# wfus/Fully-Homomorphic-Image-Processing

Measured on AMD Instinct MI355X. Metric: encrypted 8x8 blocks/sec (homomorphic DCT+quant), higher is better.
Workload: dtype f64

## Files before the change

fully-homomorphic-image-processing_amd/csrc/dct_fused.hip:

```cpp
#include "internal.h"

#include <cstdlib>

#include "fp64_core.h"

#pragma clang fp contract(off)

namespace {
using namespace fp64;

template <int L, int LE> struct Shape {
    static constexpr int N = 1 << L, E = 1 << LE, TP = N >> LE, NP = (L + LE - 1) / LE, LDS_WORDS = N + (N >> LE);
};
__host__ __device__ constexpr int g_lo(int L, int LE, int p) { return (L - LE * p - LE) < 0 ? 0 : (L - LE * p - LE); }
__host__ __device__ constexpr int g_stages(int L, int LE, int p) { return (L - LE * p) > LE ? LE : (L - LE * p); }
template <int LO, int LE> __device__ __forceinline__ int g_index(int tid, int r) {
    return ((tid >> LO) << (LO + LE)) | (r << LO) | (tid & ((1 << LO) - 1));
}
template <int LO, int LE> __device__ __forceinline__ int g_pad(int j) { return j + ((j >> (LO + LE)) << LO); }

template <int L, int LE, int P> struct PassTw {
    static constexpr int LO = g_lo(L, LE, P), S = g_stages(L, LE, P), NTW = (1 << LE) - 1;
    static constexpr int rb(int u) { return (L - 1 - (LE * P + u)) - LO; }
    static constexpr int count(int u) { return 1 << (LE - 1 - rb(u)); }
    static constexpr int offset(int u) { int o = 0; for (int v = 0; v < u; v++) o += count(v); return o; }
};
template <int L, int LE, int P>
__device__ __forceinline__ void load_tw(double (&w)[(1 << LE) - 1], const double *__restrict__ tw, int tid) {
    using T = PassTw<L, LE, P>;
    const int th = (P == 0) ? 0 : (tid >> T::LO);
#pragma unroll
    for (int u = 0; u < T::S; u++) {
#pragma unroll
        for (int i = 0; i < T::count(u); i++) w[T::offset(u) + i] = tw[(1 << (LE * P + u)) + ((th << (LE - 1 - T::rb(u))) | i)];
    }
}

template <int L, int LE, int P, int M>
__device__ __forceinline__ void fwd_pass(double (&x)[M][1 << LE], const double (&w)[(1 << LE) - 1], double p, double pinv) {
    using T = PassTw<L, LE, P>;
    constexpr int E = 1 << LE, KB = (LE == 3) ? 2 : 1;
#pragma unroll
    for (int u = 0; u < T::S; u++) {
        const int rb = T::rb(u);
#pragma unroll
        for (int b0 = 0; b0 < E / 2; b0 += KB) {
            double t[KB * M], wm[KB * M];
#pragma unroll
            for (int kb = 0; kb < KB; kb++) {
                const int b = b0 + kb, r0 = ((b >> rb) << (rb + 1)) | (b & ((1 << rb) - 1)), r1 = r0 | (1 << rb);
                const double wv = w[T::offset(u) + (r0 >> (rb + 1))];
#pragma unroll
                for (int m = 0; m < M; m++) { t[kb * M + m] = x[m][r1]; wm[kb * M + m] = wv; }
            }
            mmv<KB * M>(t, wm, p, pinv);
#pragma unroll
            for (int kb = 0; kb < KB; kb++) {
                const int b = b0 + kb, r0 = ((b >> rb) << (rb + 1)) | (b & ((1 << rb) - 1)), r1 = r0 | (1 << rb);
#pragma unroll
                for (int m = 0; m < M; m++) {
                    const double X = x[m][r0];
                    x[m][r0] = X + t[kb * M + m];
                    x[m][r1] = X - t[kb * M + m];
                }
            }
        }
    }
}

template <int L, int LE, int P, int M>
__device__ __forceinline__ void inv_pass(double (&x)[M][1 << LE], const double (&w)[(1 << LE) - 1], double ninv, double p, double pinv) {
    using T = PassTw<L, LE, P>;
    constexpr int E = 1 << LE, KB = (LE == 3) ? 2 : 1;
#pragma unroll
    for (int u = T::S - 1; u >= 0; u--) {
        const int sigma = LE * P + u, rb = T::rb(u);
        if (sigma == 0) {
#pragma unroll
            for (int b = 0; b < E / 2; b++) {
                const int r0 = ((b >> rb) << (rb + 1)) | (b & ((1 << rb) - 1)), r1 = r0 | (1 << rb);
                const double wv = w[T::offset(u) + (r0 >> (rb + 1))];
                double t[2 * M], wm[2 * M];
#pragma unroll
                for (int m = 0; m < M; m++) {
                    const double X = x[m][r0], Y = x[m][r1];
                    t[m] = X + Y; wm[m] = ninv;
                    t[M + m] = X - Y; wm[M + m] = wv;
                }
                mmv<2 * M>(t, wm, p, pinv);
#pragma unroll
                for (int m = 0; m < M; m++) { x[m][r0] = t[m]; x[m][r1] = t[M + m]; }
            }
        } else {
#pragma unroll
            for (int b0 = 0; b0 < E / 2; b0 += KB) {
                double t[KB * M], wm[KB * M];
#pragma unroll
                for (int kb = 0; kb < KB; kb++) {
                    const int b = b0 + kb, r0 = ((b >> rb) << (rb + 1)) | (b & ((1 << rb) - 1)), r1 = r0 | (1 << rb);
                    const double wv = w[T::offset(u) + (r0 >> (rb + 1))];
#pragma unroll
                    for (int m = 0; m < M; m++) {
                        const double X = x[m][r0], Y = x[m][r1];
                        x[m][r0] = X + Y;
                        t[kb * M + m] = X - Y; wm[kb * M + m] = wv;
                    }
                }
                mmv<KB * M>(t, wm, p, pinv);
#pragma unroll
                for (int kb = 0; kb < KB; kb++) {
                    const int b = b0 + kb, r0 = ((b >> rb) << (rb + 1)) | (b & ((1 << rb) - 1)), r1 = r0 | (1 << rb);
#pragma unroll
                    for (int m = 0; m < M; m++) x[m][r1] = t[kb * M + m];
                }
            }
        }
    }
}

template <int L, int LE, int LO_FROM, int LO_TO, int M>
__device__ __forceinline__ void transpose(double (&x)[M][1 << LE], double *lds, int tid, int &phase) {
    constexpr int PL = imin(LO_FROM, LO_TO), E = 1 << LE;
    constexpr bool WAVE_LOCAL = (Shape<L, LE>::TP <= 64) || (LO_FROM <= 6 && LO_TO <= 6);
#pragma unroll
    for (int m = 0; m < M; m++) {
        double *buf = lds + (phase & 1) * Shape<L, LE>::LDS_WORDS;
        phase++;
#pragma unroll
        for (int r = 0; r < E; r++) buf[g_pad<PL, LE>(g_index<LO_FROM, LE>(tid, r))] = x[m][r];
        if constexpr (WAVE_LOCAL) {
            __builtin_amdgcn_fence(__ATOMIC_RELEASE, "wavefront");
            __builtin_amdgcn_wave_barrier();
            __builtin_amdgcn_fence(__ATOMIC_ACQUIRE, "wavefront");
        } else {
            __syncthreads();
        }
#pragma unroll
        for (int r = 0; r < E; r++) x[m][r] = buf[g_pad<PL, LE>(g_index<LO_TO, LE>(tid, r))];
    }
}

template <int L, int LE, int M, typename PRE, int P = 0>
__device__ __forceinline__ void ntt_fwd(double (&x)[M][1 << LE], double (&w)[(1 << LE) - 1], const double *__restrict__ tw, double p, double pinv,
                                        double *lds, int tid, int &phase, PRE pre) {
    if constexpr (P + 1 < Shape<L, LE>::NP) {
        double wn[(1 << LE) - 1];
        if (LE >= 4) load_tw<L, LE, P + 1>(wn, tw, tid);
        fwd_pass<L, LE, P, M>(x, w, p, pinv);
        if (LE < 4) load_tw<L, LE, P + 1>(wn, tw, tid);
        if constexpr (P + 2 == Shape<L, LE>::NP) pre();
        transpose<L, LE, g_lo(L, LE, P), g_lo(L, LE, P + 1), M>(x, lds, tid, phase);
        ntt_fwd<L, LE, M, PRE, P + 1>(x, wn, tw, p, pinv, lds, tid, phase, pre);
    } else {
        fwd_pass<L, LE, P, M>(x, w, p, pinv);
    }
}
template <int L, int LE, int M, bool BIG, int P = Shape<L, LE>::NP - 1>
__device__ __forceinline__ void ntt_inv(double (&x)[M][1 << LE], double (&w)[(1 << LE) - 1], const double *__restrict__ itw, double p, double pinv,
                                        double *lds, int tid, int &phase) {
    if constexpr (P > 0) {
        double wn[(1 << LE) - 1];
        if (LE >= 4) load_tw<L, LE, P - 1>(wn, itw, tid);
        inv_pass<L, LE, P, M>(x, w, 0.0, p, pinv);
        if (LE < 4) load_tw<L, LE, P - 1>(wn, itw, tid);
        if constexpr (BIG) {
#pragma unroll
            for (int m = 0; m < M; m++)
#pragma unroll
                for (int r = 0; r < (1 << LE); r++) x[m][r] = red(x[m][r], p, pinv);
        }
        transpose<L, LE, g_lo(L, LE, P), g_lo(L, LE, P - 1), M>(x, lds, tid, phase);
        ntt_inv<L, LE, M, BIG, P - 1>(x, wn, itw, p, pinv, lds, tid, phase);
    } else {
        inv_pass<L, LE, P, M>(x, w, itw[0], p, pinv);
    }
}

constexpr double PACK_BIAS = 6755399441055744.0;
template <int E, int TP>
__device__ __forceinline__ void store_packed(u64 *__restrict__ o, const double (&x)[E]) {
    static_assert(E == 8, "packed layout is defined for 8 values per thread");
    u32 lo[8], hi[8];
#pragma unroll
    for (int r = 0; r < 8; r++) {
        const double t = x[r] + PACK_BIAS;
        lo[r] = (u32)__double2loint(t);
        hi[r] = (u32)__double2hiint(t);
    }
#pragma unroll
    for (int q = 0; q < 4; q++) o[q * TP] = (u64)lo[2 * q] | ((u64)lo[2 * q + 1] << 32);
    u32 h[2];
#pragma unroll
    for (int g = 0; g < 2; g++) {
        const u32 p01 = __builtin_amdgcn_perm(hi[4 * g + 1], hi[4 * g + 0], 0x0c0c0400u);
        const u32 p23 = __builtin_amdgcn_perm(hi[4 * g + 3], hi[4 * g + 2], 0x0c0c0400u);
        h[g] = __builtin_amdgcn_perm(p23, p01, 0x05040100u);
    }
    o[4 * TP] = (u64)h[0] | ((u64)h[1] << 32);
}
typedef __attribute__((address_space(1))) const void lc_gptr;
typedef __attribute__((address_space(3))) void lc_lptr;
template <int NT>
__device__ __forceinline__ void stage_consts(const char *ubase, u32 voff, size_t cstride_bytes, double *stg, int lane) {
#pragma unroll
    for (int i0 = 0; i0 < NT; i0 += 2) {
        const int i = (i0 + 1 < NT) ? i0 : NT - 2;
        const char *b = ubase + (size_t)i * cstride_bytes;
        __builtin_amdgcn_global_load_lds((lc_gptr *)(b + voff), (lc_lptr *)(stg + i * 64), 16, 0, 0);
    }
}

template <int L, int LE, bool BIG, int HALF, bool PACK, bool LDSC>
__device__ __forceinline__ void rows_body(const u64 *__restrict__ in, double *__restrict__ mid, const double *__restrict__ consts,
                                          const double *__restrict__ tw, const Work &wk, double p, double pinv, u32 k, double *lds) {
    using SH = Shape<L, LE>;
    constexpr int N = SH::N, TP = SH::TP, E = SH::E, NC = HalfC<HALF>::NC, FIRST = HalfC<HALF>::FIRST;
    const int tid = threadIdx.x;
    const size_t poly_words = (size_t)k * N, ct_words = 2 * poly_words;
    const size_t base = ((size_t)wk.blk * 64 + 8 * wk.line) * ct_words + (size_t)wk.poly * poly_words + (size_t)wk.prime * N;
    double w0[E - 1];
    load_tw<L, LE, 0>(w0, tw, tid);
    double x[4][E];
    constexpr u64 OFF = 1ULL << 48;
    u64 ra[2][E], rb[2][E];
    auto issue = [&](int m) {
        const u64 *a = in + base + (size_t)m * ct_words + tid, *b = in + base + (size_t)(7 - m) * ct_words + tid;
#pragma unroll
        for (int r = 0; r < E; r++) {
            ra[m & 1][r] = a[r * TP];
            rb[m & 1][r] = b[r * TP];
        }
    };
    auto combine = [&](int m) {
#pragma unroll
        for (int r = 0; r < E; r++) {
            const u64 A = ra[m & 1][r], B = rb[m & 1][r];
            x[m][r] = HALF ? u52_to_f64(A + OFF - B) - (double)OFF : u52_to_f64(A + B);
        }
    };
    if constexpr (LE >= 4) {
        issue(0);
        issue(1);
        asm volatile("" ::: "memory");
        combine(0);
        issue(2);
        asm volatile("" ::: "memory");
        combine(1);
        issue(3);
        asm volatile("" ::: "memory");
        combine(2);
        combine(3);
    } else {
#pragma unroll
        for (int m = 0; m < 4; m++) {
            issue(m);
            combine(m);
            asm volatile("" ::: "memory");
        }
    }
    const double *cp = consts + (size_t)FIRST * k * N + (size_t)wk.prime * N + tid;
    const size_t cstride = (size_t)k * N;
    double cn[9];
    auto fetch = [&](int r) {
#pragma unroll
        for (int i = 0; i < NC; i++) cn[i] = cp[(size_t)i * cstride + r * TP];
    };
    int phase = 0;
    ntt_fwd<L, LE, 4>(x, w0, tw, p, pinv, lds, tid, phase, [&] { if (LE >= 4) fetch(0); });
    const int lane = tid & 63;
    double *stg = lds + (tid >> 6) * (2 * NC * 64);
    const char *sbase = (const char *)(consts + (size_t)FIRST * cstride + (size_t)wk.prime * N);
    const u32 svoff = (u32)(((size_t)(lane >> 5) * cstride + (tid & ~63) + 2 * (lane & 31)) * sizeof(double));
    constexpr int NDMA = (NC + 1) / 2;
    if constexpr (LDSC) {
        __syncthreads();
        stage_consts<NC>(sbase, svoff, cstride * sizeof(double), stg, lane);
    }
#pragma unroll
    for (int r = 0; r < E; r++) {
        double c[9];
        if constexpr (LDSC) {
            if (r + 1 < E) stage_consts<NC>(sbase + (size_t)(r + 1) * TP * sizeof(double), svoff, cstride * sizeof(double), stg + ((r + 1) & 1) * NC * 64, lane);
            if (r + 1 < E) asm volatile("s_waitcnt vmcnt(%0)" ::"n"(NDMA) : "memory");
            else asm volatile("s_waitcnt vmcnt(0)" ::: "memory");
            const double *sr = stg + (r & 1) * NC * 64 + lane;
#pragma unroll
            for (int i = 0; i < NC; i++) c[i] = sr[i * 64];
        } else {
        if (LE < 4) fetch(r);
#pragma unroll
        for (int i = 0; i < NC; i++) c[i] = cn[i];
        if (LE >= 4 && r + 1 < E) fetch(r + 1);
        }
        line_half<HALF>(x[0][r], x[1][r], x[2][r], x[3][r], c, p, pinv);
        if (BIG) {
#pragma unroll
            for (int m = 0; m < 4; m++) x[m][r] = red(x[m][r], p, pinv);
        } else if (PACK && HALF == 0) {
            x[0][r] = red(x[0][r], p, pinv);
            x[2][r] = red(x[2][r], p, pinv);
        }
        if constexpr (LDSC) asm volatile("" ::"v"(x[0][r]), "v"(x[1][r]), "v"(x[2][r]), "v"(x[3][r]) : "memory");
    }
#pragma unroll
    for (int m = 0; m < 4; m++) {
        double *o = mid + base + (size_t)(2 * m + HALF) * ct_words + tid;
        if constexpr (PACK) {
            store_packed<E, TP>((u64 *)o, x[m]);
        } else {
#pragma unroll
            for (int r = 0; r < E; r++) o[r * TP] = x[m][r];
        }
    }
}

__host__ __device__ constexpr int occ_waves(int tp, int lds_words) {
    return ((2 * lds_words * 16 <= 160 * 1024) ? 2 : 1) * tp / 256 < 1 ? 1 : ((2 * lds_words * 16 <= 160 * 1024) ? 2 : 1) * tp / 256;
}
template <int L, int LE> struct Occ { static constexpr int W = occ_waves(Shape<L, LE>::TP, Shape<L, LE>::LDS_WORDS); };

template <int L, int LE, bool BIG, bool PACK, bool LDSC>
__global__ __launch_bounds__((Shape<L, LE>::TP), (Occ<L, LE>::W)) void k_dct_rows(const u64 *__restrict__ in, double *__restrict__ mid,
                                                                  const double *__restrict__ consts, const double *__restrict__ tw_all,
                                                                  const Modulus *__restrict__ mods, u32 k) {
    __shared__ double lds[2 * Shape<L, LE>::LDS_WORDS];
    const Work wk = decode(blockIdx.x, k);
    const double p = (double)mods[wk.prime].q, pinv = 1.0 / p;
    const double *tw = tw_all + (size_t)wk.prime * Shape<L, LE>::N;
    if (wk.half) rows_body<L, LE, BIG, 1, PACK, LDSC>(in, mid, consts, tw, wk, p, pinv, k, lds);
    else rows_body<L, LE, BIG, 0, PACK, LDSC>(in, mid, consts, tw, wk, p, pinv, k, lds);
}

template <int L, int LE, bool BIG, int HALF, bool PACK>
__device__ __forceinline__ void cols_body(const double *__restrict__ mid, u64 *__restrict__ out, const double *__restrict__ consts,
                                          const double *__restrict__ itw, const Work &wk, double p, double pinv, u32 k, double *lds) {
    using SH = Shape<L, LE>;
    constexpr int N = SH::N, TP = SH::TP, E = SH::E, NC = HalfC<HALF>::NC, FIRST = HalfC<HALF>::FIRST;
    constexpr int LASTP = SH::NP - 1;
    const int tid = threadIdx.x;
    const size_t poly_words = (size_t)k * N, ct_words = 2 * poly_words;
    const size_t base = ((size_t)wk.blk * 64 + wk.line) * ct_words + (size_t)wk.poly * poly_words + (size_t)wk.prime * N;
    const size_t row_stride = 8 * ct_words;
    const size_t cstride = (size_t)k * N;
    const double *cp = consts + (size_t)FIRST * cstride + (size_t)wk.prime * N + tid;
    const double *sp = consts + (size_t)(12 + 8 * HALF + wk.line) * cstride + (size_t)wk.prime * N + tid;
    double cn[9], sn[4];
    auto fetch = [&](int r) {
#pragma unroll
        for (int i = 0; i < NC; i++) cn[i] = cp[(size_t)i * cstride + r * TP];
#pragma unroll
        for (int m = 0; m < 4; m++) sn[m] = sp[(size_t)(16 * m) * cstride + r * TP];
    };
    double wl[E - 1];
    if constexpr (!PACK) {
        fetch(0);
        load_tw<L, LE, LASTP>(wl, itw, tid);
    }
    double x[4][E];
    if constexpr (PACK) {
        u64 wa[4][5], wb[4][5];
#pragma unroll
        for (int m = 0; m < 4; m++) {
            const u64 *a = (const u64 *)(mid + base + (size_t)m * row_stride) + tid, *b = (const u64 *)(mid + base + (size_t)(7 - m) * row_stride) + tid;
#pragma unroll
            for (int q = 0; q < 5; q++) { wa[m][q] = a[q * TP]; wb[m][q] = b[q * TP]; }
        }
#pragma unroll
        for (int m = 0; m < 4; m++) {
#pragma unroll
            for (int r = 0; r < E; r++) {
                const u32 la = (r & 1) ? (u32)(wa[m][r >> 1] >> 32) : (u32)wa[m][r >> 1];
                const u32 lb = (r & 1) ? (u32)(wb[m][r >> 1] >> 32) : (u32)wb[m][r >> 1];
                const u32 hwa = (r & 4) ? (u32)(wa[m][4] >> 32) : (u32)wa[m][4], hwb = (r & 4) ? (u32)(wb[m][4] >> 32) : (u32)wb[m][4];
                const double ta = __hiloint2double((int)(0x43380000u + (u32)(int)(signed char)(hwa >> (8 * (r & 3)))), (int)la);
                const double tb = __hiloint2double((int)(0x43380000u + (u32)(int)(signed char)(hwb >> (8 * (r & 3)))), (int)lb);
                x[m][r] = HALF ? ta - tb : ta + (tb - 2.0 * PACK_BIAS);
            }
        }
    } else {
#pragma unroll
        for (int m = 0; m < 4; m++) {
            const double *a = mid + base + (size_t)m * row_stride + tid, *b = mid + base + (size_t)(7 - m) * row_stride + tid;
#pragma unroll
            for (int r = 0; r < E; r++) {
                const double A = a[r * TP], B = b[r * TP];
                x[m][r] = HALF ? A - B : A + B;
            }
        }
    }
    if constexpr (PACK) load_tw<L, LE, LASTP>(wl, itw, tid);
#pragma unroll
    for (int r = 0; r < E; r++) {
        double c[9], sc[4];
        if (PACK) fetch(r);
#pragma unroll
        for (int i = 0; i < NC; i++) c[i] = cn[i];
#pragma unroll
        for (int m = 0; m < 4; m++) sc[m] = sn[m];
        if (!PACK && r + 1 < E) fetch(r + 1);
        line_half<HALF>(x[0][r], x[1][r], x[2][r], x[3][r], c, p, pinv);
        double y[4] = {x[0][r], x[1][r], x[2][r], x[3][r]};
        mmv<4>(y, sc, p, pinv);
#pragma unroll
        for (int m = 0; m < 4; m++) x[m][r] = y[m];
    }
    int phase = 0;
    ntt_inv<L, LE, 4, BIG>(x, wl, itw, p, pinv, lds, tid, phase);
#pragma unroll
    for (int m = 0; m < 4; m++) {
        u64 *o = out + base + (size_t)(2 * m + HALF) * row_stride + tid;
#pragma unroll
        for (int r = 0; r < E; r++) {
            double v = x[m][r];
            v = v < 0.0 ? v + p : v;
            o[r * TP] = f64_to_u52(v);
        }
    }
}

template <int L, int LE, bool BIG, bool PACK>
__global__ __launch_bounds__((Shape<L, LE>::TP), (Occ<L, LE>::W)) void k_dct_cols(const double *__restrict__ mid, u64 *__restrict__ out,
                                                                  const double *__restrict__ consts, const double *__restrict__ itw_all,
                                                                  const Modulus *__restrict__ mods, u32 k) {
    __shared__ double lds[2 * Shape<L, LE>::LDS_WORDS];
    const Work wk = decode(blockIdx.x, k);
    const double p = (double)mods[wk.prime].q, pinv = 1.0 / p;
    const double *itw = itw_all + (size_t)wk.prime * Shape<L, LE>::N;
    if (wk.half) cols_body<L, LE, BIG, 1, PACK>(mid, out, consts, itw, wk, p, pinv, k, lds);
    else cols_body<L, LE, BIG, 0, PACK>(mid, out, consts, itw, wk, p, pinv, k, lds);
}

template <int L, int LE>
__global__ __launch_bounds__((Shape<L, LE>::TP), (Occ<L, LE>::W)) void k_dct_one_launch(const u64 *__restrict__ in, double *__restrict__ mid, u64 *__restrict__ out,
                                                                        const double *__restrict__ consts, const double *__restrict__ tw_all,
                                                                        const double *__restrict__ itw_all, const Modulus *__restrict__ mods, u32 k,
                                                                        u32 n_blocks, u32 dist, u32 *__restrict__ arrived, u32 *__restrict__ err) {
    __shared__ double lds[2 * Shape<L, LE>::LDS_WORDS];
    const u32 xcd = blockIdx.x & 7, seq = blockIdx.x >> 3, chunk = seq >> 5, r = seq & 31;
    const bool is_row = r < 16;
    const long j = is_row ? (long)chunk : (long)chunk - (long)(dist & 0xffffu);
    const u32 n_units = n_blocks * 2 * k;
    if (j < 0) return;
    const u64 g = (u64)j * 8 + xcd;
    if (g >= n_units) return;
    Work wk;
    wk.prime = (u32)(g / (n_blocks * 2));
    const u32 rem = (u32)(g - (u64)wk.prime * n_blocks * 2);
    wk.blk = rem >> 1;
    wk.poly = rem & 1;
    wk.line = (r & 15) >> 1;
    wk.half = r & 1;
    const double p = (double)mods[wk.prime].q, pinv = 1.0 / p;
    if (is_row) {
        const double *tw = tw_all + (size_t)wk.prime * Shape<L, LE>::N;
        if (wk.half) rows_body<L, LE, false, 1, true, true>(in, mid, consts, tw, wk, p, pinv, k, lds);
        else rows_body<L, LE, false, 0, true, true>(in, mid, consts, tw, wk, p, pinv, k, lds);
        if (dist & 0x10000u) return;
        __syncthreads();
        if (threadIdx.x == 0) {
            __threadfence();
            atomicAdd(arrived + g, 1u);
        }
    } else {
        if (!(dist & 0x10000u) && threadIdx.x == 0) {
            u32 spins = 0;
            while (__hip_atomic_load(arrived + g, __ATOMIC_RELAXED, __HIP_MEMORY_SCOPE_AGENT) < 16u) {
                __builtin_amdgcn_s_sleep(8);
                if (++spins > (1u << 24)) { atomicExch(err, 1u); break; }
            }
            __threadfence();
        }
        __syncthreads();
        const double *itw = itw_all + (size_t)wk.prime * Shape<L, LE>::N;
        if (wk.half) cols_body<L, LE, false, 1, true>(mid, out, consts, itw, wk, p, pinv, k, lds);
        else cols_body<L, LE, false, 0, true>(mid, out, consts, itw, wk, p, pinv, k, lds);
    }
}

__global__ void k_consts_to_f64(const ulonglong2 *__restrict__ in, double *__restrict__ out, const Modulus *__restrict__ mods, u32 k, u32 n, u32 le, u32 total) {
    const u32 i = blockIdx.x * blockDim.x + threadIdx.x;
    if (i >= total) return;
    const u32 pos = i % n, rowbase = i - pos;
    const u32 tp = n >> le, r = pos / tp, t = pos % tp;
    const u32 j = (t << le) + r;
    const u32 src = (j & 15) * (n >> 4) + (j >> 4);
    const u64 q = mods[(i / n) % k].q;
    const u64 w = in[rowbase + src].x;
    out[i] = w > q / 2 ? -(double)(q - w) : (double)w;
}

template <int L, int LE>
__global__ __launch_bounds__((Shape<L, LE>::TP), (Occ<L, LE>::W)) void k_rgb2ycc_f64(u64 *__restrict__ R, u64 *__restrict__ G, u64 *__restrict__ Bc,
                                                                     const double *__restrict__ consts, const double *__restrict__ tw_all,
                                                                     const double *__restrict__ itw_all, const Modulus *__restrict__ mods,
                                                                     const u64 *__restrict__ yoff, u32 yoff_len, u32 k, u32 group, u64 gstride) {
    using SH = Shape<L, LE>;
    constexpr int N = SH::N, TP = SH::TP, E = SH::E, LASTP = SH::NP - 1;
    __shared__ double lds[2 * SH::LDS_WORDS];
    const int tid = threadIdx.x;
    const u32 per_prime = gridDim.x / k;
    const u32 prime = blockIdx.x / per_prime;
    const u32 pp = blockIdx.x - prime * per_prime;
    const u32 poly = pp & 1, pix = pp >> 1;
    const u64 q = mods[prime].q;
    const double p = (double)q, pinv = 1.0 / p;
    const double *tw = tw_all + (size_t)prime * N, *itw = itw_all + (size_t)prime * N;
    const size_t pix_off = group ? (size_t)(pix / group) * gstride + (size_t)(pix % group) * 2 * k * N : (size_t)pix * 2 * k * N;
    const size_t off = pix_off + ((size_t)poly * k + prime) * N + tid;
    double w0[E - 1];
    load_tw<L, LE, 0>(w0, tw, tid);
    double x[3][E];
    {
        const u64 *src[3] = {R + off, G + off, Bc + off};
#pragma unroll
        for (int m = 0; m < 3; m++)
#pragma unroll
            for (int r = 0; r < E; r++) x[m][r] = u52_to_f64(src[m][r * TP]);
    }
    int phase = 0;
    ntt_fwd<L, LE, 3>(x, w0, tw, p, pinv, lds, tid, phase, [] {});
    double wl[E - 1];
    load_tw<L, LE, LASTP>(wl, itw, tid);
    const double *cp = consts + (size_t)prime * N + tid;
    const size_t cstride = (size_t)k * N;
#pragma unroll
    for (int r = 0; r < E; r++) {
        double c[9], y[9];
#pragma unroll
        for (int i = 0; i < 9; i++) { c[i] = cp[(size_t)i * cstride + r * TP]; y[i] = x[i % 3][r]; }
        mmv<9>(y, c, p, pinv);
        x[0][r] = y[0] + y[1] + y[2];
        x[1][r] = y[3] - y[4] + y[5];
        x[2][r] = y[6] - y[7] - y[8];
    }
    ntt_inv<L, LE, 3, false>(x, wl, itw, p, pinv, lds, tid, phase);
    u64 *dst[3] = {R + off, G + off, Bc + off};
#pragma unroll
    for (int m = 0; m < 3; m++)
#pragma unroll
        for (int r = 0; r < E; r++) {
            double v = x[m][r];
            v = v < 0.0 ? v + p : v;
            u64 o = f64_to_u52(v);
            if (m == 0 && poly == 0) {
                const u32 j = (u32)(r * TP + tid);
                if (j < yoff_len) o = submod(o, yoff[(size_t)prime * yoff_len + j], q);
            }
            dst[m][r * TP] = o;
        }
}

template <int L, int LE, int M, int MODE>
__global__ __launch_bounds__((Shape<L, LE>::TP), (Occ<L, LE>::W)) void k_poly_f64(const u64 *__restrict__ in, u64 *__restrict__ out,
                                                                  const ulonglong2 *__restrict__ plain, const double *__restrict__ tw_all,
                                                                  const double *__restrict__ itw_all, const Modulus *__restrict__ mods, u32 k) {
    using SH = Shape<L, LE>;
    constexpr int N = SH::N, TP = SH::TP, E = SH::E, LASTP = SH::NP - 1;
    static_assert(LE == 3, "slot-order mapping below is written for 8 values per thread");
    __shared__ double lds[2 * SH::LDS_WORDS];
    const int tid = threadIdx.x;
    const u32 per_prime = gridDim.x / k;
    const u32 prime = blockIdx.x / per_prime;
    const u32 g = blockIdx.x - prime * per_prime;
    const double p = (double)mods[prime].q, pinv = 1.0 / p;
    const double *tw = tw_all + (size_t)prime * N, *itw = itw_all + (size_t)prime * N;
    const int slot0 = ((tid & 1) << 3) * (N >> 4) + (tid >> 1);
    double x[M][E];
    int phase = 0;
    if constexpr (MODE != 1) {
        double w0[E - 1];
        load_tw<L, LE, 0>(w0, tw, tid);
#pragma unroll
        for (int m = 0; m < M; m++) {
            const u64 *src = in + ((size_t)(g * M + m) * k + prime) * N + tid;
#pragma unroll
            for (int r = 0; r < E; r++) x[m][r] = u52_to_f64(src[r * TP]);
        }
        ntt_fwd<L, LE, M>(x, w0, tw, p, pinv, lds, tid, phase, [] {});
    } else {
#pragma unroll
        for (int m = 0; m < M; m++) {
            const u64 *src = in + ((size_t)(g * M + m) * k + prime) * N + slot0;
#pragma unroll
            for (int r = 0; r < E; r++) x[m][r] = u52_to_f64(src[r * (N >> 4)]);
        }
    }
    if constexpr (MODE == 0) {
#pragma unroll
        for (int m = 0; m < M; m++) {
            u64 *dst = out + ((size_t)(g * M + m) * k + prime) * N + slot0;
#pragma unroll
            for (int r = 0; r < E; r++) {
                double v = red(x[m][r], p, pinv);
                v = v < 0.0 ? v + p : v;
                dst[r * (N >> 4)] = f64_to_u52(v);
            }
        }
        return;
    }
    double wl[E - 1];
    load_tw<L, LE, LASTP>(wl, itw, tid);
    if constexpr (MODE == 2) {
        const ulonglong2 *pp = plain + (size_t)prime * N + slot0;
#pragma unroll
        for (int r = 0; r < E; r++) {
            const double w = u52_to_f64(pp[r * (N >> 4)].x);
            double y[M], wm[M];
#pragma unroll
            for (int m = 0; m < M; m++) { y[m] = x[m][r]; wm[m] = w; }
            mmv<M>(y, wm, p, pinv);
#pragma unroll
            for (int m = 0; m < M; m++) x[m][r] = y[m];
        }
    }
    ntt_inv<L, LE, M, false>(x, wl, itw, p, pinv, lds, tid, phase);
#pragma unroll
    for (int m = 0; m < M; m++) {
        u64 *dst = out + ((size_t)(g * M + m) * k + prime) * N + tid;
#pragma unroll
        for (int r = 0; r < E; r++) {
            double v = x[m][r];
            v = v < 0.0 ? v + p : v;
            dst[r * TP] = f64_to_u52(v);
        }
    }
}

}


static u32 dct_shape_le(const fhe_ctx *c) {
    if (c->opt.dct_le != 3) return 4;
    if (c->logn == 12 && c->max_prime_bits <= 40) return 3;
    if (c->logn == 13 || c->logn == 11) return 3;
    return 4;
}

bool fhe_dct_f64_supported(const fhe_ctx *c) {
    return c && c->qb.d_tw_f64 && c->max_prime_bits <= 47 && (c->logn >= 10 && c->logn <= 13);
}

int fhe_dct_f64_make_consts(const fhe_ctx *c, fhe_dct_plan *plan, hipStream_t st) {
    const u32 total = DCT_NCONST * c->k * c->n;
    HIP_TRY(hipMalloc(&plan->d_consts_f64, sizeof(double) * total));
    const u32 le = dct_shape_le(c);
    k_consts_to_f64<<<(total + 255) / 256, 256, 0, st>>>(plan->d_consts, plan->d_consts_f64, c->qb.d_mod, c->k, c->n, le, total);
    KERNEL_CHECK();
    return FHE_OK;
}



template <int L, int LE>
static void launch_pair(const fhe_ctx *c, const fhe_dct_plan *plan, const u64 *in, u64 *out, double *mid, unsigned grid, bool big, hipStream_t st, int which) {
    constexpr int TP = Shape<L, LE>::TP;
    if constexpr (LE == 4) {
        if (big) {
            if (which & 1) k_dct_rows<L, LE, true, false, false><<<grid, TP, 0, st>>>(in, mid, plan->d_consts_f64, c->qb.d_tw_f64, c->qb.d_mod, c->k);
            if (which & 2) k_dct_cols<L, LE, true, false><<<grid, TP, 0, st>>>(mid, out, plan->d_consts_f64, c->qb.d_itw_f64, c->qb.d_mod, c->k);
            return;
        }
    }
    if constexpr (LE == 3) {
        if (big) {
            if (which & 1) k_dct_rows<L, LE, true, false, false><<<grid, TP, 0, st>>>(in, mid, plan->d_consts_f64, c->qb.d_tw_f64, c->qb.d_mod, c->k);
            if (which & 2) k_dct_cols<L, LE, true, false><<<grid, TP, 0, st>>>(mid, out, plan->d_consts_f64, c->qb.d_itw_f64, c->qb.d_mod, c->k);
            return;
        }
        if (c->max_prime_bits <= 37 && c->opt.dct_pack) {
            if (which & 1) {
                if (c->opt.dct_ldsc) k_dct_rows<L, LE, false, true, true><<<grid, TP, 0, st>>>(in, mid, plan->d_consts_f64, c->qb.d_tw_f64, c->qb.d_mod, c->k);
                else k_dct_rows<L, LE, false, true, false><<<grid, TP, 0, st>>>(in, mid, plan->d_consts_f64, c->qb.d_tw_f64, c->qb.d_mod, c->k);
            }
            if (which & 2) k_dct_cols<L, LE, false, true><<<grid, TP, 0, st>>>(mid, out, plan->d_consts_f64, c->qb.d_itw_f64, c->qb.d_mod, c->k);
            return;
        }
    }
    {
        if (which & 1) k_dct_rows<L, LE, false, false, false><<<grid, TP, 0, st>>>(in, mid, plan->d_consts_f64, c->qb.d_tw_f64, c->qb.d_mod, c->k);
        if (which & 2) k_dct_cols<L, LE, false, false><<<grid, TP, 0, st>>>(mid, out, plan->d_consts_f64, c->qb.d_itw_f64, c->qb.d_mod, c->k);
    }
}

int fhe_dct_f64_launch(const fhe_ctx *c, const fhe_dct_plan *plan, const u64 *in, u64 *out, u64 n_blocks, double *mid, hipStream_t st, int which) {
    const u64 items = n_blocks * 8 * 2 * c->k;
    const u64 grid = items * 2;
    if (grid > 0x7fffffffULL) return fail(FHE_ERR_PARAM, "too many blocks for one launch");
    const bool big = c->max_prime_bits > 40;
    if (c->opt.dct_one_launch && which == 3 && c->logn == 12 && dct_shape_le(c) == 3 && c->max_prime_bits <= 37 && c->opt.dct_pack && c->d_arrived) {
        const u64 n_units = n_blocks * 2 * c->k;
        if (n_units > c->arrived_cap) return fail(FHE_ERR_PARAM, "one-launch experiment: wave too large for the arrival counters");
        HIP_TRY(hipMemsetAsync(c->d_arrived, 0, (n_units + 1) * sizeof(u32), st));
        const u32 dist = c->opt.dct_one_launch;
        const u64 chunks = (n_units + 7) / 8 + (dist & 0xffffu);
        k_dct_one_launch<12, 3><<<(unsigned)(chunks * 32 * 8), Shape<12, 3>::TP, 0, st>>>(in, mid, out, plan->d_consts_f64, c->qb.d_tw_f64, c->qb.d_itw_f64, c->qb.d_mod,
                                                                                       c->k, (u32)n_blocks, dist, c->d_arrived + 1, c->d_arrived);
        KERNEL_CHECK();
        u32 timed_out = 0;
        HIP_TRY(hipMemcpyAsync(&timed_out, c->d_arrived, sizeof(u32), hipMemcpyDeviceToHost, st));
        HIP_TRY(hipStreamSynchronize(st));
        if (timed_out) return fail(FHE_ERR_HIP, "one-launch experiment: a column workgroup timed out waiting for its row transforms; the output is incomplete");
        return FHE_OK;
    }
    switch (c->logn) {
        case 10: launch_pair<10, 4>(c, plan, in, out, mid, (unsigned)grid, big, st, which); break;
        case 11: launch_pair<11, 3>(c, plan, in, out, mid, (unsigned)grid, big, st, which); break;
        case 12: if (dct_shape_le(c) == 3) launch_pair<12, 3>(c, plan, in, out, mid, (unsigned)grid, false, st, which); else launch_pair<12, 4>(c, plan, in, out, mid, (unsigned)grid, big, st, which); break;
        case 13: if (dct_shape_le(c) == 3) launch_pair<13, 3>(c, plan, in, out, mid, (unsigned)grid, big, st, which); else launch_pair<13, 4>(c, plan, in, out, mid, (unsigned)grid, big, st, which); break;
        default: return fail(FHE_ERR_PARAM, "fused FP64 path supports n in {1024, 2048, 4096, 8192}");
    }
    KERNEL_CHECK();
    return FHE_OK;
}

bool fhe_rgb_f64_supported(const fhe_ctx *c) {
    return fhe_dct_f64_supported(c) && c->logn == 12 && c->max_prime_bits <= 40;
}

int fhe_rgb_f64_make_consts(const fhe_ctx *c, const ulonglong2 *d_c, double **out, hipStream_t st) {
    const u32 total = 9 * c->k * c->n;
    HIP_TRY(hipMalloc(out, sizeof(double) * total));
    k_consts_to_f64<<<(total + 255) / 256, 256, 0, st>>>(d_c, *out, c->qb.d_mod, c->k, c->n, 3, total);
    KERNEL_CHECK();
    return FHE_OK;
}

int fhe_rgb_f64_launch(const fhe_ctx *c, u64 *r, u64 *g, u64 *b, u64 count, const double *consts, const u64 *yoff, u32 yoff_len, hipStream_t st, u32 group, u64 gstride) {
    const u64 grid = count * 2 * c->k;
    if (grid > 0x7fffffffULL) return fail(FHE_ERR_PARAM, "too many pixels for one launch");
    k_rgb2ycc_f64<12, 3><<<(unsigned)grid, Shape<12, 3>::TP, 0, st>>>(r, g, b, consts, c->qb.d_tw_f64, c->qb.d_itw_f64, c->qb.d_mod, yoff, yoff_len, c->k, group, gstride);
    KERNEL_CHECK();
    return FHE_OK;
}

int fhe_poly_f64_launch(int mode, const fhe_ctx *c, const u64 *in, u64 *out, u64 n_polys, const ulonglong2 *plain, hipStream_t st) {
    const u64 grid2 = (n_polys / 2) * c->k, grid1 = n_polys * c->k;
    if (grid1 > 0x7fffffffULL) return fail(FHE_ERR_PARAM, "too many polynomials for one launch");
    constexpr int TP = Shape<12, 3>::TP;
#define LAUNCH_POLY(M, GRID)                                                                                                          \
    switch (mode) {                                                                                                                   \
        case 0: k_poly_f64<12, 3, M, 0><<<(unsigned)(GRID), TP, 0, st>>>(in, out, plain, c->qb.d_tw_f64, c->qb.d_itw_f64, c->qb.d_mod, c->k); break; \
        case 1: k_poly_f64<12, 3, M, 1><<<(unsigned)(GRID), TP, 0, st>>>(in, out, plain, c->qb.d_tw_f64, c->qb.d_itw_f64, c->qb.d_mod, c->k); break; \
        default: k_poly_f64<12, 3, M, 2><<<(unsigned)(GRID), TP, 0, st>>>(in, out, plain, c->qb.d_tw_f64, c->qb.d_itw_f64, c->qb.d_mod, c->k); break; \
    }
    if (n_polys % 2 == 0) { LAUNCH_POLY(2, grid2) } else { LAUNCH_POLY(1, grid1) }
#undef LAUNCH_POLY
    KERNEL_CHECK();
    return FHE_OK;
}

namespace {
using namespace fp64;

template <int HALF>
__device__ __forceinline__ void idct_half(double (&v)[4], const double (&c)[12], double p, double pinv) {
    if constexpr (HALF == 0) {
        double y[3] = {v[1] + v[3], v[3], v[1]};
        const double w[3] = {c[0], c[2], c[1]};
        mmv<3>(y, w, p, pinv);
        const double t2 = y[0] + y[1], t3 = y[0] + y[2], t0 = v[0] + v[2], t1 = v[0] - v[2];
        v[0] = t0 + t3;
        v[1] = t1 + t2;
        v[2] = t1 - t2;
        v[3] = t0 - t3;
    } else {
        const double u0 = v[3], u1 = v[2], u2 = v[1], u3 = v[0];
        const double z1 = u0 + u3, z2 = u1 + u2, z3 = u0 + u2, z4 = u1 + u3;
        double ya[5] = {z3 + z4, u0, u1, u2, u3}, yb[4] = {z1, z2, z3, z4};
        const double wa[5] = {c[3], c[4], c[5], c[6], c[7]}, wb[4] = {c[8], c[9], c[10], c[11]};
        mmv<5>(ya, wa, p, pinv);
        mmv<4>(yb, wb, p, pinv);
        const double z3b = yb[2] + ya[0], z4b = yb[3] + ya[0];
        v[0] = ya[4] + yb[0] + z4b;
        v[1] = ya[3] + yb[1] + z3b;
        v[2] = ya[2] + yb[1] + z4b;
        v[3] = ya[1] + yb[0] + z3b;
    }
}

template <int L, int LE, int HALF>
__device__ __forceinline__ void irows_body(const u64 *__restrict__ in, double *__restrict__ mid, const double *__restrict__ consts,
                                           const double *__restrict__ tw, const Work &wk, double p, double pinv, u32 k, double *lds) {
    using SH = Shape<L, LE>;
    constexpr int N = SH::N, TP = SH::TP, E = SH::E;
    const int tid = threadIdx.x;
    const size_t poly_words = (size_t)k * N, ct_words = 2 * poly_words, cstride = (size_t)k * N;
    const size_t base = ((size_t)wk.blk * 64 + 8 * wk.line) * ct_words + (size_t)wk.poly * poly_words + (size_t)wk.prime * N + tid;
    double w0[E - 1];
    load_tw<L, LE, 0>(w0, tw, tid);
    double x[4][E];
#pragma unroll
    for (int m = 0; m < 4; m++) {
        const u64 *a = in + base + (size_t)(2 * m + HALF) * ct_words;
#pragma unroll
        for (int r = 0; r < E; r++) x[m][r] = u52_to_f64(a[r * TP]);
        asm volatile("" ::: "memory");
    }
    int phase = 0;
    ntt_fwd<L, LE, 4>(x, w0, tw, p, pinv, lds, tid, phase, [] {});
    const double *cp = consts + (size_t)wk.prime * N + tid;
#pragma unroll
    for (int r = 0; r < E; r++) {
        double c[12], s[4], v[4];
#pragma unroll
        for (int i = 0; i < 12; i++) c[i] = cp[(size_t)i * cstride + r * TP];
#pragma unroll
        for (int m = 0; m < 4; m++) {
            s[m] = cp[(size_t)(12 + 8 * wk.line + 2 * m + HALF) * cstride + r * TP];
            v[m] = red(x[m][r], p, pinv);
        }
        mmv<4>(v, s, p, pinv);
        idct_half<HALF>(v, c, p, pinv);
#pragma unroll
        for (int m = 0; m < 4; m++) x[m][r] = red(v[m], p, pinv);
    }
#pragma unroll
    for (int m = 0; m < 4; m++) {
        double *o = mid + base + (size_t)(4 * HALF + m) * ct_words;
#pragma unroll
        for (int r = 0; r < E; r++) o[r * TP] = x[m][r];
    }
}

template <int L, int LE>
__global__ __launch_bounds__((Shape<L, LE>::TP), (Occ<L, LE>::W)) void k_idct_rows(const u64 *__restrict__ in, double *__restrict__ mid,
                                                                   const double *__restrict__ consts, const double *__restrict__ tw_all,
                                                                   const Modulus *__restrict__ mods, u32 k) {
    __shared__ double lds[2 * Shape<L, LE>::LDS_WORDS];
    const Work wk = decode(blockIdx.x, k);
    const double p = (double)mods[wk.prime].q, pinv = 1.0 / p;
    const double *tw = tw_all + (size_t)wk.prime * Shape<L, LE>::N;
    if (wk.half) irows_body<L, LE, 1>(in, mid, consts, tw, wk, p, pinv, k, lds);
    else irows_body<L, LE, 0>(in, mid, consts, tw, wk, p, pinv, k, lds);
}

template <int L, int LE, bool BIG, int HALF>
__device__ __forceinline__ void icols_body(const double *__restrict__ mid, u64 *__restrict__ out, const double *__restrict__ consts,
                                           const double *__restrict__ itw, const Work &wk, double p, double pinv, u32 k, double *lds) {
    using SH = Shape<L, LE>;
    constexpr int N = SH::N, TP = SH::TP, E = SH::E, LASTP = SH::NP - 1;
    const int tid = threadIdx.x;
    const size_t poly_words = (size_t)k * N, ct_words = 2 * poly_words, cstride = (size_t)k * N;
    const size_t base = (size_t)wk.blk * 64 * ct_words + (size_t)wk.poly * poly_words + (size_t)wk.prime * N + tid;
    const u32 col = wk.line, m = col < 4 ? col : 7 - col;
    const bool neg = col >= 4;
    const double *cp = consts + (size_t)wk.prime * N + tid;
    double x[4][E];
#pragma unroll
    for (int r = 0; r < E; r++) {
        double d[8], c[12];
#pragma unroll
        for (int rr = 0; rr < 8; rr++) {
            const double A = mid[base + (size_t)(8 * rr + m) * ct_words + r * TP], B = mid[base + (size_t)(8 * rr + 4 + m) * ct_words + r * TP];
            d[rr] = neg ? A - B : A + B;
        }
#pragma unroll
        for (int i = 0; i < 12; i++) c[i] = cp[(size_t)i * cstride + r * TP];
        double ev[4] = {d[0], d[2], d[4], d[6]}, od[4] = {d[1], d[3], d[5], d[7]};
        idct_half<0>(ev, c, p, pinv);
        idct_half<1>(od, c, p, pinv);
#pragma unroll
        for (int j = 0; j < 4; j++) x[j][r] = red(HALF ? ev[3 - j] - od[3 - j] : ev[j] + od[j], p, pinv);
    }
    double wl[E - 1];
    load_tw<L, LE, LASTP>(wl, itw, tid);
    int phase = 0;
    ntt_inv<L, LE, 4, BIG>(x, wl, itw, p, pinv, lds, tid, phase);
#pragma unroll
    for (int j = 0; j < 4; j++) {
        u64 *o = out + base + (size_t)(8 * (4 * HALF + j) + col) * ct_words;
#pragma unroll
        for (int r = 0; r < E; r++) {
            double v = x[j][r];
            v = v < 0.0 ? v + p : v;
            o[r * TP] = f64_to_u52(v);
        }
    }
}

template <int L, int LE, bool BIG>
__global__ __launch_bounds__((Shape<L, LE>::TP), (Occ<L, LE>::W)) void k_idct_cols(const double *__restrict__ mid, u64 *__restrict__ out,
                                                                   const double *__restrict__ consts, const double *__restrict__ itw_all,
                                                                   const Modulus *__restrict__ mods, u32 k) {
    __shared__ double lds[2 * Shape<L, LE>::LDS_WORDS];
    const Work wk = decode(blockIdx.x, k);
    const double p = (double)mods[wk.prime].q, pinv = 1.0 / p;
    const double *itw = itw_all + (size_t)wk.prime * Shape<L, LE>::N;
    if (wk.half) icols_body<L, LE, BIG, 1>(mid, out, consts, itw, wk, p, pinv, k, lds);
    else icols_body<L, LE, BIG, 0>(mid, out, consts, itw, wk, p, pinv, k, lds);
}

template <int L, int LE>
void launch_ipair(const fhe_ctx *c, const double *consts, const u64 *in, u64 *out, double *mid, unsigned grid, bool big, hipStream_t st) {
    constexpr int TP = Shape<L, LE>::TP;
    k_idct_rows<L, LE><<<grid, TP, 0, st>>>(in, mid, consts, c->qb.d_tw_f64, c->qb.d_mod, c->k);
    if (big) k_idct_cols<L, LE, true><<<grid, TP, 0, st>>>(mid, out, consts, c->qb.d_itw_f64, c->qb.d_mod, c->k);
    else k_idct_cols<L, LE, false><<<grid, TP, 0, st>>>(mid, out, consts, c->qb.d_itw_f64, c->qb.d_mod, c->k);
}
}

int fhe_idct_f64_make_consts(const fhe_ctx *c, const ulonglong2 *d_consts, double **out, hipStream_t st) {
    const u32 total = DCT_NCONST * c->k * c->n;
    HIP_TRY(hipMalloc(out, sizeof(double) * total));
    k_consts_to_f64<<<(total + 255) / 256, 256, 0, st>>>(d_consts, *out, c->qb.d_mod, c->k, c->n, dct_shape_le(c), total);
    KERNEL_CHECK();
    return FHE_OK;
}

int fhe_idct_f64_launch(const fhe_ctx *c, const double *consts, const u64 *in, u64 *out, u64 n_blocks, double *mid, hipStream_t st) {
    const u64 grid = n_blocks * 8 * 2 * c->k * 2;
    if (grid > 0x7fffffffULL) return fail(FHE_ERR_PARAM, "too many blocks for one launch");
    const bool big = c->max_prime_bits > 40;
    switch (c->logn) {
        case 10: launch_ipair<10, 4>(c, consts, in, out, mid, (unsigned)grid, big, st); break;
        case 11: launch_ipair<11, 3>(c, consts, in, out, mid, (unsigned)grid, big, st); break;
        case 12: if (dct_shape_le(c) == 3) launch_ipair<12, 3>(c, consts, in, out, mid, (unsigned)grid, big, st); else launch_ipair<12, 4>(c, consts, in, out, mid, (unsigned)grid, big, st); break;
        case 13: if (dct_shape_le(c) == 3) launch_ipair<13, 3>(c, consts, in, out, mid, (unsigned)grid, big, st); else launch_ipair<13, 4>(c, consts, in, out, mid, (unsigned)grid, big, st); break;
        default: return fail(FHE_ERR_PARAM, "fused FP64 path supports n in {1024, 2048, 4096, 8192}");
    }
    KERNEL_CHECK();
    return FHE_OK;
}
```

fully-homomorphic-image-processing_amd/csrc/fp64_core.h:

```cpp
#pragma once
#include "internal.h"

#pragma clang fp contract(off)

namespace fp64 {

__device__ __forceinline__ double mm(double y, double w, double p, double pinv) {
    const double h = y * w;
    const double l = __builtin_fma(y, w, -h);
    const double q = __builtin_rint(h * pinv);
    return __builtin_fma(-q, p, h) + l;
}
__device__ __forceinline__ double red(double x, double p, double pinv) {
    return __builtin_fma(-__builtin_rint(x * pinv), p, x);
}
template <int K>
__device__ __forceinline__ void mmv(double (&y)[K], const double (&w)[K], double p, double pinv) {
    double h[K], l[K], q[K];
#pragma unroll
    for (int i = 0; i < K; i++) h[i] = y[i] * w[i];
#pragma unroll
    for (int i = 0; i < K; i++) q[i] = h[i] * pinv;
#pragma unroll
    for (int i = 0; i < K; i++) l[i] = __builtin_fma(y[i], w[i], -h[i]);
#pragma unroll
    for (int i = 0; i < K; i++) q[i] = __builtin_rint(q[i]);
#pragma unroll
    for (int i = 0; i < K; i++) h[i] = __builtin_fma(-q[i], p, h[i]);
#pragma unroll
    for (int i = 0; i < K; i++) y[i] = h[i] + l[i];
}

__device__ __forceinline__ double u52_to_f64(u64 v) { return __longlong_as_double((long long)(v | 0x4330000000000000ULL)) - 4503599627370496.0; }
__device__ __forceinline__ u64 f64_to_u52(double v) { return (u64)__double_as_longlong(v + 4503599627370496.0) & 0x000FFFFFFFFFFFFFULL; }

template <int HALF>
__device__ __forceinline__ void line_half(double &x0, double &x1, double &x2, double &x3, const double (&c)[9], double p, double pinv) {
    if constexpr (HALF == 0) {
        const double tmp10 = x0 + x3, tmp13 = x0 - x3, tmp11 = x1 + x2, tmp12 = x1 - x2;
        double y[3] = {tmp12 + tmp13, tmp13, tmp12};
        const double w[3] = {c[0], c[1], c[2]};
        mmv<3>(y, w, p, pinv);
        x0 = tmp10 + tmp11;
        x2 = tmp10 - tmp11;
        x1 = y[0] + y[1];
        x3 = y[0] + y[2];
    } else {
        const double tmp7 = x0, tmp6 = x1, tmp5 = x2, tmp4 = x3;
        const double z1 = tmp4 + tmp7, z2 = tmp5 + tmp6, z3 = tmp4 + tmp6, z4 = tmp5 + tmp7;
        double ya[5] = {z3 + z4, tmp4, tmp5, tmp6, tmp7}, yb[4] = {z1, z2, z3, z4};
        const double wa[5] = {c[0], c[1], c[2], c[3], c[4]}, wb[4] = {c[5], c[6], c[7], c[8]};
        mmv<5>(ya, wa, p, pinv);
        mmv<4>(yb, wb, p, pinv);
        const double y[9] = {ya[0], ya[1], ya[2], ya[3], ya[4], yb[0], yb[1], yb[2], yb[3]};
        const double z3b = y[7] + y[0], z4b = y[8] + y[0];
        x0 = y[4] + y[5] + z4b;
        x1 = y[3] + y[6] + z3b;
        x2 = y[2] + y[6] + z4b;
        x3 = y[1] + y[5] + z3b;
    }
}
template <int HALF> struct HalfC { static constexpr int NC = HALF ? 9 : 3, FIRST = HALF ? 3 : 0; };

struct Work { u32 blk, line, poly, prime, half; };
__device__ __forceinline__ Work decode(u32 idx, u32 k) {
    const u32 w = ((idx >> 4) << 3) | (idx & 7);
    const u32 per_prime = (gridDim.x >> 1) / k;
    Work o;
    o.half = (idx >> 3) & 1;
    o.prime = w / per_prime;
    u32 t = w - o.prime * per_prime;
    o.poly = t & 1;
    t >>= 1;
    o.line = t & 7;
    o.blk = t >> 3;
    return o;
}


}
```

Baseline: 81450.

## Use buffer-resource loads and stores with scalar offsets in fused DCT kernels

Global pointer arithmetic for the input, mid, constant and output arrays is replaced with AMDGPU buffer resource descriptors. Each access becomes a per-thread vector offset plus a uniform scalar offset, which is meant to cut 64-bit VGPR address computation and register pressure. The constant staging now uses buffer_load_lds instead of global_load_lds. Two small arithmetic simplifications are also added: a biased u52 subtraction and a fused conditional-add residue conversion. A new guard rejects problem sizes that exceed the 32-bit offset window.

After: 84230, median of 6. 3.4% higher.

```diff
diff --git a/fully-homomorphic-image-processing_amd/csrc/dct_fused.hip b/fully-homomorphic-image-processing_amd/csrc/dct_fused.hip
--- a/fully-homomorphic-image-processing_amd/csrc/dct_fused.hip
+++ b/fully-homomorphic-image-processing_amd/csrc/dct_fused.hip
@@ -178,7 +178,7 @@
 
 constexpr double PACK_BIAS = 6755399441055744.0;
 template <int E, int TP>
-__device__ __forceinline__ void store_packed(u64 *__restrict__ o, const double (&x)[E]) {
+__device__ __forceinline__ void store_packed(char *__restrict__ ob, u32 vo, u32 so, const double (&x)[E]) {
     static_assert(E == 8, "packed layout is defined for 8 values per thread");
     u32 lo[8], hi[8];
 #pragma unroll
@@ -188,7 +188,7 @@
         hi[r] = (u32)__double2hiint(t);
     }
 #pragma unroll
-    for (int q = 0; q < 4; q++) o[q * TP] = (u64)lo[2 * q] | ((u64)lo[2 * q + 1] << 32);
+    for (int q = 0; q < 4; q++) *(u64 *)(ob + (size_t)(so + q * TP * 8) + vo) = (u64)lo[2 * q] | ((u64)lo[2 * q + 1] << 32);
     u32 h[2];
 #pragma unroll
     for (int g = 0; g < 2; g++) {
@@ -196,17 +196,15 @@
         const u32 p23 = __builtin_amdgcn_perm(hi[4 * g + 3], hi[4 * g + 2], 0x0c0c0400u);
         h[g] = __builtin_amdgcn_perm(p23, p01, 0x05040100u);
     }
-    o[4 * TP] = (u64)h[0] | ((u64)h[1] << 32);
-}
-typedef __attribute__((address_space(1))) const void lc_gptr;
+    *(u64 *)(ob + (size_t)(so + 4 * TP * 8) + vo) = (u64)h[0] | ((u64)h[1] << 32);
+}
 typedef __attribute__((address_space(3))) void lc_lptr;
 template <int NT>
-__device__ __forceinline__ void stage_consts(const char *ubase, u32 voff, size_t cstride_bytes, double *stg, int lane) {
+__device__ __forceinline__ void stage_consts(gwin_t w, u32 voff, u32 soff, u32 cstride_bytes, double *stg) {
 #pragma unroll
     for (int i0 = 0; i0 < NT; i0 += 2) {
         const int i = (i0 + 1 < NT) ? i0 : NT - 2;
-        const char *b = ubase + (size_t)i * cstride_bytes;
-        __builtin_amdgcn_global_load_lds((lc_gptr *)(b + voff), (lc_lptr *)(stg + i * 64), 16, 0, 0);
+        __builtin_amdgcn_raw_ptr_buffer_load_lds(w, (lc_lptr *)(stg + i * 64), 16, voff, soff + (u32)i * cstride_bytes, 0, 0);
     }
 }
 
@@ -218,24 +216,24 @@
     const int tid = threadIdx.x;
     const size_t poly_words = (size_t)k * N, ct_words = 2 * poly_words;
     const size_t base = ((size_t)wk.blk * 64 + 8 * wk.line) * ct_words + (size_t)wk.poly * poly_words + (size_t)wk.prime * N;
+    const gwin_t win_in = gwin(in + base), win_mid = gwin(mid + base);
+    const u32 vo = (u32)tid * 8u, ctb = (u32)(ct_words * 8);
     double w0[E - 1];
     load_tw<L, LE, 0>(w0, tw, tid);
     double x[4][E];
-    constexpr u64 OFF = 1ULL << 48;
     u64 ra[2][E], rb[2][E];
     auto issue = [&](int m) {
-        const u64 *a = in + base + (size_t)m * ct_words + tid, *b = in + base + (size_t)(7 - m) * ct_words + tid;
 #pragma unroll
         for (int r = 0; r < E; r++) {
-            ra[m & 1][r] = a[r * TP];
-            rb[m & 1][r] = b[r * TP];
+            ra[m & 1][r] = gld_u64(win_in, vo, (u32)m * ctb + r * TP * 8);
+            rb[m & 1][r] = gld_u64(win_in, vo, (u32)(7 - m) * ctb + r * TP * 8);
         }
     };
     auto combine = [&](int m) {
 #pragma unroll
         for (int r = 0; r < E; r++) {
             const u64 A = ra[m & 1][r], B = rb[m & 1][r];
-            x[m][r] = HALF ? u52_to_f64(A + OFF - B) - (double)OFF : u52_to_f64(A + B);
+            x[m][r] = HALF ? u52_biased(A) - u52_biased(B) : u52_to_f64(A + B);
         }
     };
     if constexpr (LE >= 4) {
@@ -258,29 +256,30 @@
             asm volatile("" ::: "memory");
         }
     }
-    const double *cp = consts + (size_t)FIRST * k * N + (size_t)wk.prime * N + tid;
     const size_t cstride = (size_t)k * N;
+    const gwin_t win_c = gwin(consts + (size_t)FIRST * cstride + (size_t)wk.prime * N);
+    const u32 csb = (u32)(cstride * 8);
     double cn[9];
     auto fetch = [&](int r) {
 #pragma unroll
-        for (int i = 0; i < NC; i++) cn[i] = cp[(size_t)i * cstride + r * TP];
+        for (int i = 0; i < NC; i++) cn[i] = gld_f64(win_c, vo, (u32)i * csb + r * TP * 8);
     };
     int phase = 0;
     ntt_fwd<L, LE, 4>(x, w0, tw, p, pinv, lds, tid, phase, [&] { if (LE >= 4) fetch(0); });
     const int lane = tid & 63;
     double *stg = lds + (tid >> 6) * (2 * NC * 64);
-    const char *sbase = (const char *)(consts + (size_t)FIRST * cstride + (size_t)wk.prime * N);
     const u32 svoff = (u32)(((size_t)(lane >> 5) * cstride + (tid & ~63) + 2 * (lane & 31)) * sizeof(double));
     constexpr int NDMA = (NC + 1) / 2;
     if constexpr (LDSC) {
+        __builtin_amdgcn_sched_barrier(0);
         __syncthreads();
-        stage_consts<NC>(sbase, svoff, cstride * sizeof(double), stg, lane);
+        stage_consts<NC>(win_c, svoff, 0, csb, stg);
     }
 #pragma unroll
     for (int r = 0; r < E; r++) {
         double c[9];
         if constexpr (LDSC) {
-            if (r + 1 < E) stage_consts<NC>(sbase + (size_t)(r + 1) * TP * sizeof(double), svoff, cstride * sizeof(double), stg + ((r + 1) & 1) * NC * 64, lane);
+            if (r + 1 < E) stage_consts<NC>(win_c, svoff, (r + 1) * TP * 8, csb, stg + ((r + 1) & 1) * NC * 64);
             if (r + 1 < E) asm volatile("s_waitcnt vmcnt(%0)" ::"n"(NDMA) : "memory");
             else asm volatile("s_waitcnt vmcnt(0)" ::: "memory");
             const double *sr = stg + (r & 1) * NC * 64 + lane;
@@ -304,12 +303,12 @@
     }
 #pragma unroll
     for (int m = 0; m < 4; m++) {
-        double *o = mid + base + (size_t)(2 * m + HALF) * ct_words + tid;
+        const u32 so = (u32)(2 * m + HALF) * ctb;
         if constexpr (PACK) {
-            store_packed<E, TP>((u64 *)o, x[m]);
+            store_packed<E, TP>((char *)(mid + base), vo, so, x[m]);
         } else {
 #pragma unroll
-            for (int r = 0; r < E; r++) o[r * TP] = x[m][r];
+            for (int r = 0; r < E; r++) gst_f64(win_mid, vo, so + r * TP * 8, x[m][r]);
         }
     }
 }
@@ -340,16 +339,18 @@
     const int tid = threadIdx.x;
     const size_t poly_words = (size_t)k * N, ct_words = 2 * poly_words;
     const size_t base = ((size_t)wk.blk * 64 + wk.line) * ct_words + (size_t)wk.poly * poly_words + (size_t)wk.prime * N;
-    const size_t row_stride = 8 * ct_words;
     const size_t cstride = (size_t)k * N;
-    const double *cp = consts + (size_t)FIRST * cstride + (size_t)wk.prime * N + tid;
-    const double *sp = consts + (size_t)(12 + 8 * HALF + wk.line) * cstride + (size_t)wk.prime * N + tid;
+    const gwin_t win_mid = gwin(mid + base), win_out = gwin(out + base);
+    const gwin_t win_c = gwin(consts + (size_t)FIRST * cstride + (size_t)wk.prime * N);
+    const gwin_t win_s = gwin(consts + (size_t)(12 + 8 * HALF + wk.line) * cstride + (size_t)wk.prime * N);
+    const u32 vo = (u32)tid * 8u, rsb = (u32)(ct_words * 64), csb = (u32)(cstride * 8);
+    const double pbias = p + 4503599627370496.0;
     double cn[9], sn[4];
     auto fetch = [&](int r) {
 #pragma unroll
-        for (int i = 0; i < NC; i++) cn[i] = cp[(size_t)i * cstride + r * TP];
-#pragma unroll
-        for (int m = 0; m < 4; m++) sn[m] = sp[(size_t)(16 * m) * cstride + r * TP];
+        for (int i = 0; i < NC; i++) cn[i] = gld_f64(win_c, vo, (u32)i * csb + r * TP * 8);
+#pragma unroll
+        for (int m = 0; m < 4; m++) sn[m] = gld_f64(win_s, vo, (u32)(16 * m) * csb + r * TP * 8);
     };
     double wl[E - 1];
     if constexpr (!PACK) {
@@ -361,9 +362,11 @@
         u64 wa[4][5], wb[4][5];
 #pragma unroll
         for (int m = 0; m < 4; m++) {
-            const u64 *a = (const u64 *)(mid + base + (size_t)m * row_stride) + tid, *b = (const u64 *)(mid + base + (size_t)(7 - m) * row_stride) + tid;
-#pragma unroll
-            for (int q = 0; q < 5; q++) { wa[m][q] = a[q * TP]; wb[m][q] = b[q * TP]; }
+#pragma unroll
+            for (int q = 0; q < 5; q++) {
+                wa[m][q] = gld_u64(win_mid, vo, (u32)m * rsb + q * TP * 8);
+                wb[m][q] = gld_u64(win_mid, vo, (u32)(7 - m) * rsb + q * TP * 8);
+            }
         }
 #pragma unroll
         for (int m = 0; m < 4; m++) {
@@ -380,10 +383,9 @@
     } else {
 #pragma unroll
         for (int m = 0; m < 4; m++) {
-            const double *a = mid + base + (size_t)m * row_stride + tid, *b = mid + base + (size_t)(7 - m) * row_stride + tid;
 #pragma unroll
             for (int r = 0; r < E; r++) {
-                const double A = a[r * TP], B = b[r * TP];
+                const double A = gld_f64(win_mid, vo, (u32)m * rsb + r * TP * 8), B = gld_f64(win_mid, vo, (u32)(7 - m) * rsb + r * TP * 8);
                 x[m][r] = HALF ? A - B : A + B;
             }
         }
@@ -408,13 +410,8 @@
     ntt_inv<L, LE, 4, BIG>(x, wl, itw, p, pinv, lds, tid, phase);
 #pragma unroll
     for (int m = 0; m < 4; m++) {
-        u64 *o = out + base + (size_t)(2 * m + HALF) * row_stride + tid;
-#pragma unroll
-        for (int r = 0; r < E; r++) {
-            double v = x[m][r];
-            v = v < 0.0 ? v + p : v;
-            o[r * TP] = f64_to_u52(v);
-        }
+#pragma unroll
+        for (int r = 0; r < E; r++) gst_u64(win_out, vo, (u32)(2 * m + HALF) * rsb + r * TP * 8, f64_to_residue(x[m][r], pbias));
     }
 }
 
@@ -686,6 +683,7 @@
     const u64 items = n_blocks * 8 * 2 * c->k;
     const u64 grid = items * 2;
     if (grid > 0x7fffffffULL) return fail(FHE_ERR_PARAM, "too many blocks for one launch");
+    if ((u64)c->k * c->n >= (1ULL << 21)) return fail(FHE_ERR_PARAM, "fused FP64 path: a block of ciphertexts exceeds the 2 GiB addressing window");
     const bool big = c->max_prime_bits > 40;
     if (c->opt.dct_one_launch && which == 3 && c->logn == 12 && dct_shape_le(c) == 3 && c->max_prime_bits <= 37 && c->opt.dct_pack && c->d_arrived) {
         const u64 n_units = n_blocks * 2 * c->k;
diff --git a/fully-homomorphic-image-processing_amd/csrc/fp64_core.h b/fully-homomorphic-image-processing_amd/csrc/fp64_core.h
--- a/fully-homomorphic-image-processing_amd/csrc/fp64_core.h
+++ b/fully-homomorphic-image-processing_amd/csrc/fp64_core.h
@@ -33,6 +33,20 @@
 
 __device__ __forceinline__ double u52_to_f64(u64 v) { return __longlong_as_double((long long)(v | 0x4330000000000000ULL)) - 4503599627370496.0; }
 __device__ __forceinline__ u64 f64_to_u52(double v) { return (u64)__double_as_longlong(v + 4503599627370496.0) & 0x000FFFFFFFFFFFFFULL; }
+__device__ __forceinline__ double u52_biased(u64 v) { return __longlong_as_double((long long)(v | 0x4330000000000000ULL)); }
+__device__ __forceinline__ u64 f64_to_residue(double v, double pbias) {
+    return (u64)__double_as_longlong(v + (v < 0.0 ? pbias : 4503599627370496.0)) & 0x000FFFFFFFFFFFFFULL;
+}
+
+typedef u32 u32x2 __attribute__((ext_vector_type(2)));
+typedef __amdgpu_buffer_rsrc_t gwin_t;
+__device__ __forceinline__ gwin_t gwin(const void *base) {
+    return __builtin_amdgcn_make_buffer_rsrc(const_cast<void *>(base), 0, -1, 0x00020000 );
+}
+__device__ __forceinline__ u64 gld_u64(gwin_t w, u32 voff, u32 soff) { return __builtin_bit_cast(u64, __builtin_amdgcn_raw_buffer_load_b64(w, voff, soff, 0)); }
+__device__ __forceinline__ double gld_f64(gwin_t w, u32 voff, u32 soff) { return __builtin_bit_cast(double, __builtin_amdgcn_raw_buffer_load_b64(w, voff, soff, 0)); }
+__device__ __forceinline__ void gst_u64(gwin_t w, u32 voff, u32 soff, u64 v) { __builtin_amdgcn_raw_buffer_store_b64(__builtin_bit_cast(u32x2, v), w, voff, soff, 0); }
+__device__ __forceinline__ void gst_f64(gwin_t w, u32 voff, u32 soff, double v) { __builtin_amdgcn_raw_buffer_store_b64(__builtin_bit_cast(u32x2, v), w, voff, soff, 0); }
 
 template <int HALF>
 __device__ __forceinline__ void line_half(double &x0, double &x1, double &x2, double &x3, const double (&c)[9], double p, double pinv) {
```
